# jvde-github/AIS-catcher

Hardware: NVIDIA H100
Metric: IQ MSamples/s through full 2-ch demod chain (higher is better)
Workload: dtype f32

## Files before the change

ais-catcher_b200/csrc/fe_stream.cuh:

```cuda
#pragma once
#include "exact.cuh"
#include "params.h"
#include <atomic>
#include <algorithm>

namespace aisgpu {

struct Cic5 { c64 h0, h1, h2, h3, h4; };
__device__ __forceinline__ void cic5_zero(Cic5 &s) { s.h0 = s.h1 = s.h2 = s.h3 = s.h4 = 0ull; }
__device__ __forceinline__ c64 ds2_pair(Cic5 &s, c64 xe, c64 xo, c64 sc) {
	c64 z = xe;
	const c64 r0 = z; z = padd(z, s.h0);
	const c64 r1 = z; z = padd(z, s.h1);
	const c64 r2 = z; z = padd(z, s.h2);
	const c64 r3 = z; z = padd(z, s.h3);
	const c64 r4 = z; z = padd(z, s.h4);
	const c64 out = pmul(z, sc);
	z = xo;
	s.h0 = z; z = padd(z, r0);
	s.h1 = z; z = padd(z, r1);
	s.h2 = z; z = padd(z, r2);
	s.h3 = z; z = padd(z, r3);
	s.h4 = z;
	(void)r4;
	return out;
}
__device__ __forceinline__ void fcic_pair(Cic5 &s, c64 xe, c64 xo, c64 sc, c64 &oe, c64 &oo) {
	c64 z = xe;
	const c64 r0 = z; z = padd(z, s.h0);
	const c64 r1 = z; z = padd(z, s.h1);
	const c64 r2 = z; z = padd(z, s.h2);
	const c64 r3 = z; z = padd(z, s.h3);
	const c64 r4 = z; z = padd(z, s.h4);
	oe = pmul(z, sc);
	z = xo;
	s.h0 = z; z = padd(z, r0);
	s.h1 = z; z = padd(z, r1);
	s.h2 = z; z = padd(z, r2);
	s.h3 = z; z = padd(z, r3);
	s.h4 = z; z = padd(z, r4);
	oo = pmul(z, sc);
}
struct Cic5u { uint32_t h0, h1, h2, h3, h4; };
__device__ __forceinline__ void cic5u_zero(Cic5u &s) { s.h0 = s.h1 = s.h2 = s.h3 = s.h4 = 0u; }
template <int SHIFT>
__device__ __forceinline__ uint32_t ds2u_pair(Cic5u &s, uint32_t xe, uint32_t xo) {
	constexpr uint32_t m16 = 0xFFFFu >> SHIFT, mask = m16 | (m16 << 16);
	uint32_t z = xe;
	const uint32_t r0 = z; z += s.h0;
	const uint32_t r1 = z; z += s.h1;
	const uint32_t r2 = z; z += s.h2;
	const uint32_t r3 = z; z += s.h3;
	z += s.h4;
	const uint32_t out = (z >> SHIFT) & mask;
	z = xo;
	s.h0 = z; z += r0;
	s.h1 = z; z += r1;
	s.h2 = z; z += r2;
	s.h3 = z; z += r3;
	s.h4 = z;
	return out;
}
__device__ __forceinline__ c64 u16pair_to_c64(uint32_t z) {
	z ^= 0x80008000u;
	return pack2(__fmul_rn((float)(short)(z & 0xFFFFu), 3.0517578125e-05f), __fmul_rn((float)(short)(z >> 16), 3.0517578125e-05f));
}

template <int FMT, int G>
struct StFmt {
	static constexpr int BPS = FMT == 0 ? 8 : (FMT == 3 ? 4 : 2);
	static constexpr int CHUNK = G * BPS;
	static constexpr int PIECES = CHUNK / 16;
	static constexpr int SLOT = CHUNK + 16;
};
template <int FMT>
__device__ __forceinline__ void st_read_pair(const unsigned char *slot, int j, c64 &xe, c64 &xo) {
	if (FMT == 0) {
		const ulonglong2 v = *reinterpret_cast<const ulonglong2 *>(slot + j * 16);
		xe = v.x;
		xo = v.y;
	}
	else if (FMT == 1) {
		const uchar4 v = *reinterpret_cast<const uchar4 *>(slot + j * 4);
		xe = pack2(__fmul_rn((float)((int)v.x - 128), 0.0078125f), __fmul_rn((float)((int)v.y - 128), 0.0078125f));
		xo = pack2(__fmul_rn((float)((int)v.z - 128), 0.0078125f), __fmul_rn((float)((int)v.w - 128), 0.0078125f));
	}
	else if (FMT == 2) {
		const char4 v = *reinterpret_cast<const char4 *>(slot + j * 4);
		xe = pack2(__fmul_rn((float)v.x, 0.0078125f), __fmul_rn((float)v.y, 0.0078125f));
		xo = pack2(__fmul_rn((float)v.z, 0.0078125f), __fmul_rn((float)v.w, 0.0078125f));
	}
	else {
		const short4 v = *reinterpret_cast<const short4 *>(slot + j * 8);
		xe = pack2(__fmul_rn((float)v.x, 3.0517578125e-05f), __fmul_rn((float)v.y, 3.0517578125e-05f));
		xo = pack2(__fmul_rn((float)v.z, 3.0517578125e-05f), __fmul_rn((float)v.w, 3.0517578125e-05f));
	}
}

template <int FMT, int K, int ST_G, int ST_NB, int ST_WARPS, bool PRE = false>
__global__ void __launch_bounds__(ST_WARPS * 32) k_frontend_st(const FeParams p) {
	static_assert(K >= 3 && K <= 7, "streaming front end: 768 kS/s .. 12288 kS/s");
	static_assert(ST_G <= (1 << (K + 2)) && (ST_G % 16) == 0, "a chunk must not be longer than a super-step");
	typedef StFmt<FMT, ST_G> F;
	constexpr int SS = 1 << (K + 2);
	constexpr int NCH = SS / ST_G;
	constexpr int N96 = SS >> K;
	extern __shared__ __align__(16) unsigned char st_ring[];
	const int lane = threadIdx.x & 31, wib = threadIdx.x >> 5;
	const long long g0 = ((long long)blockIdx.x * ST_WARPS + wib) * 32;
	const int L = p.st_L;
	if (g0 >= (long long)p.st_B * L) return;
	int stream = (int)((g0 + lane) / L), sub = (int)((g0 + lane) - (long long)stream * L);
	const bool ghost = stream >= p.st_B;
	if (ghost) { stream = p.st_B - 1; sub = L - 1; }
	const int n_short = L - p.st_r;
	const int n_main = ghost ? 0 : p.st_q + (sub >= n_short ? 1 : 0);
	unsigned char(*ring)[32 * F::SLOT] = reinterpret_cast<unsigned char(*)[32 * F::SLOT]>(st_ring + (size_t)wib * ST_NB * 32 * F::SLOT);
	const long long a = ((long long)sub * p.st_q + max(0, sub - n_short)) * SS;
	const int n_super = p.P / SS + p.st_q + (p.st_r ? 1 : 0);
	const int warp_chunks = n_super * NCH;
	constexpr int OWN_PER_IT = 32 / F::PIECES;
	const int o0 = lane / F::PIECES, q0 = lane % F::PIECES;
	const unsigned char *in0 = reinterpret_cast<const unsigned char *>(p.in) - (long long)p.P * F::BPS;
	const unsigned my_off = (unsigned)((((long long)stream * p.in_stride + a) * F::BPS) >> 4);
	const unsigned long long my_warm = sub == 0 ? (unsigned long long)(reinterpret_cast<const unsigned char *>(p.tail) + (long long)stream * p.P * F::BPS)
												: (unsigned long long)(in0 + ((unsigned long long)my_off << 4));
	const int dst_off = o0 * F::SLOT + q0 * 16;
	unsigned own_off[F::PIECES];
#pragma unroll
	for (int it = 0; it < F::PIECES; it++) own_off[it] = __shfl_sync(0xffffffffu, my_off, it * OWN_PER_IT + o0);
	auto prefetch = [&](int c) {
		if (c < warp_chunks) {
			const long long coff = (long long)c * (ST_G * F::BPS) + q0 * 16;
			unsigned char *dst = &ring[c % ST_NB][dst_off];
			if (c * ST_G < p.P) {
#pragma unroll 1
				for (int it = 0; it < F::PIECES; it++) {
					const unsigned long long w = __shfl_sync(0xffffffffu, my_warm, it * OWN_PER_IT + o0);
					cp_async16(dst + it * OWN_PER_IT * F::SLOT, reinterpret_cast<const unsigned char *>(w) + coff);
				}
			}
			else {
				unsigned long long base = (unsigned long long)(in0 + coff);
				asm volatile("" : "+l"(base));
#pragma unroll
				for (int it = 0; it < F::PIECES; it++) cp_async16(dst + it * OWN_PER_IT * F::SLOT, reinterpret_cast<const unsigned char *>(base + ((unsigned long long)own_off[it] << 4)));
			}
		}
		cp_async_commit();
	};
	const c64 sc = pack2(0.03125f, 0.03125f);
	static_assert(FMT != 4 || (K == 4 && !PRE), "the integer front end exists for the exact 1536K bucket only (Model.cpp:222-236)");
	Cic5 lv[K], chA, chB, fA, fB;
	Cic5u lu[4];
	uint32_t pendu[4];
#pragma unroll
	for (int l = 0; l < 4; l++) { cic5u_zero(lu[l]); pendu[l] = 0u; }
#pragma unroll
	for (int l = 0; l < K; l++) cic5_zero(lv[l]);
	cic5_zero(chA); cic5_zero(chB); cic5_zero(fA); cic5_zero(fB);
	c64 fd1 = 0ull, fd2 = 0ull;
	const float2 *rot_g = PRE ? nullptr : p.rot + (p.P >> K) + ((a - p.P) >> K);
	float2 *Cg = PRE ? p.D0 + (long long)stream * p.d0_stride + p.d0_off + ((a - p.P) >> K)
					 : p.C + (long long)(stream * 2) * p.c_stride + p.c_off + ((a - p.P) >> (K + 1));
	const int warm_super = p.P / SS;
#pragma unroll
	for (int c = 0; c < ST_NB - 1; c++) prefetch(c);
	float2 rt_n1[N96], rt_n2[N96];
#pragma unroll
	for (int i = 0; i < N96; i++) {
		rt_n1[i] = PRE ? make_float2(0.f, 0.f) : __ldg(rot_g + i);
		rt_n2[i] = PRE ? make_float2(0.f, 0.f) : __ldg(rot_g + (n_super > 1 ? N96 : 0) + i);
	}
	for (int ss = 0; ss < n_super; ss++) {
		float2 rt[N96];
#pragma unroll
		for (int i = 0; i < N96; i++) {
			rt[i] = rt_n1[i];
			rt_n1[i] = rt_n2[i];
		}
		if (!PRE && ss + 2 < n_super) {
#pragma unroll
			for (int i = 0; i < N96; i++) rt_n2[i] = __ldg(rot_g + (ss + 2) * N96 + i);
		}
		c64 lvK[N96];
		c64 pend[K + 1];
		c64 upE = 0ull, dnE = 0ull, waE = 0ull, wbE = 0ull;
		c64 outA0 = 0ull, outA1 = 0ull, outB0 = 0ull, outB1 = 0ull;
#pragma unroll
		for (int cc = 0; cc < NCH; cc++) {
			const int c = ss * NCH + cc;
			prefetch(c + ST_NB - 1);
			cp_async_wait<ST_NB - 1>();
			__syncwarp();
			{
				const unsigned char *slot = &ring[c % ST_NB][lane * F::SLOT];
#pragma unroll
				for (int j = 0; j < ST_G / 2; j++) {
					const int n1 = cc * (ST_G / 2) + j;
					c64 y = 0ull;
					int idx = n1;
					bool live = true;
					if (FMT == 4) {
						const uchar4 v = *reinterpret_cast<const uchar4 *>(slot + j * 4);
						uint32_t yu = ds2u_pair<3>(lu[0], (uint32_t)v.x | ((uint32_t)v.y << 16), (uint32_t)v.z | ((uint32_t)v.w << 16));
						if ((idx & 1) == 0) { pendu[1] = yu; live = false; }
						else { yu = ds2u_pair<4>(lu[1], pendu[1], yu); idx >>= 1; }
						if (live) {
							if ((idx & 1) == 0) { pendu[2] = yu; live = false; }
							else { yu = ds2u_pair<5>(lu[2], pendu[2], yu); idx >>= 1; }
						}
						if (live) {
							if ((idx & 1) == 0) { pendu[3] = yu; live = false; }
							else {
								y = u16pair_to_c64(ds2u_pair<0>(lu[3], pendu[3], yu));
								if (p.st_first && sub == 0 && ss < warm_super) y = 0ull;
								idx >>= 1;
							}
						}
					}
					else {
						c64 xe, xo;
						st_read_pair<FMT == 4 ? 1 : FMT>(slot, j, xe, xo);
						y = ds2_pair(lv[0], xe, xo, sc);
#pragma unroll
						for (int l = 1; l < K; l++) {
							if (live) {
								if ((idx & 1) == 0) { pend[l] = y; live = false; }
								else { y = ds2_pair(lv[l], pend[l], y, sc); idx >>= 1; }
							}
						}
					}
					if (live && PRE) lvK[idx] = y;
					if (live && !PRE) {
						c64 x = y;
						if (p.use_fdc) {
							const float2 h1 = unpack2(fd1), h2 = unpack2(fd2), yv = unpack2(y);
							const float tx = __fadd_rn(h1.x, yv.x), ty = __fadd_rn(h1.y, yv.y);
							x = pack2(__fadd_rn(__fmul_rn(p.fdc_alpha, tx), __fmul_rn(h2.x, p.fdc_beta)),
									  __fadd_rn(__fmul_rn(p.fdc_alpha, ty), __fmul_rn(h2.y, p.fdc_beta)));
							fd1 = fd2;
							fd2 = y;
						}
						const float2 xv = unpack2(x);
						const float2 r = rt[idx];
						const float RR = __fmul_rn(xv.x, r.x), II = __fmul_rn(xv.y, r.y), RI = __fmul_rn(xv.x, r.y), IR = __fmul_rn(xv.y, r.x);
						const c64 up = pack2(__fsub_rn(RR, II), __fadd_rn(IR, RI));
						const c64 dn = pack2(__fadd_rn(RR, II), __fsub_rn(IR, RI));
						if ((idx & 1) == 0) { upE = up; dnE = dn; }
						else {
							const c64 wa = ds2_pair(chA, upE, up, sc), wb = ds2_pair(chB, dnE, dn, sc);
							if ((idx & 2) == 0) { waE = wa; wbE = wb; }
							else {
								fcic_pair(fA, waE, wa, sc, outA0, outA1);
								fcic_pair(fB, wbE, wb, sc, outB0, outB1);
							}
						}
					}
				}
			}
			__syncwarp();
		}
		if (PRE) {
			if (ss >= warm_super && ss - warm_super < n_main) {
				float2 *o = Cg + ss * N96;
#pragma unroll
				for (int i = 0; i < N96; i += 2) *reinterpret_cast<ulonglong2 *>(o + i) = make_ulonglong2(lvK[i], lvK[i + 1]);
			}
		}
		else if (ss >= warm_super && ss - warm_super < n_main) {
			float2 *o = Cg + ss * 2;
			*reinterpret_cast<ulonglong2 *>(o) = make_ulonglong2(outA0, outA1);
			*reinterpret_cast<ulonglong2 *>(o + p.c_stride) = make_ulonglong2(outB0, outB1);
		}
	}
	cp_async_wait<0>();
}

static inline bool st_plan(long long B, int nss, int warm, int wpc, int slots, int min_ratio, int forced_L, int &L, int &q, int &r) {
	const int q_min = warm * min_ratio > 0 ? warm * min_ratio : 1;
	if (nss < q_min) return false;
	const int L_max = nss / q_min;
	auto cost = [&](int l) {
		const long long ctas = ((B * l + 31) / 32 + wpc - 1) / wpc;
		const long long waves = (ctas + slots - 1) / slots;
		return (double)waves * ((nss + l - 1) / l + warm);
	};
	int best = 1;
	double cb = cost(1);
	for (int l = 2; l <= L_max; l++) {
		const double c = cost(l);
		if (c < cb * 0.97) { cb = c; best = l; }
	}
	if (forced_L > 0) best = forced_L < L_max ? forced_L : L_max;
	L = best;
	q = nss / L;
	r = nss - q * L;
	return true;
}
struct CtaSlots { std::atomic<int> slots{0}, sms{0}; };
template <typename Kernel>
static cudaError_t cta_slots(CtaSlots &cache, Kernel *kernel, int threads, size_t smem, int &slots, int &sms) {
	slots = cache.slots.load();
	sms = cache.sms.load();
	if (slots) return cudaSuccess;
	int dev = 0, occ = 0;
	cudaError_t e;
	if ((e = cudaGetDevice(&dev)) != cudaSuccess) return e;
	if ((e = cudaDeviceGetAttribute(&sms, cudaDevAttrMultiProcessorCount, dev)) != cudaSuccess) return e;
	if ((e = cudaOccupancyMaxActiveBlocksPerMultiprocessor(&occ, kernel, threads, smem)) != cudaSuccess) return e;
	slots = sms * (occ > 0 ? occ : 1);
	cache.sms.store(sms);
	cache.slots.store(slots);
	return cudaSuccess;
}

template <int FMT, int K, int G, int NB, int WPC, bool PRE>
static cudaError_t launch_st_one(const FeParams &p_in, int forced_L, cudaStream_t s) {
	constexpr int GG = G <= (1 << (K + 2)) ? G : (1 << (K + 2));
	constexpr int SS = 1 << (K + 2);
	const size_t smem = (size_t)WPC * NB * 32 * StFmt<FMT, GG>::SLOT;
	cudaError_t e = cudaFuncSetAttribute(k_frontend_st<FMT, K, GG, NB, WPC, PRE>, cudaFuncAttributeMaxDynamicSharedMemorySize, (int)smem);
	if (e != cudaSuccess) return e;
	static CtaSlots cache;
	int slots = 0, sms = 0;
	if ((e = cta_slots(cache, k_frontend_st<FMT, K, GG, NB, WPC, PRE>, WPC * 32, smem, slots, sms)) != cudaSuccess) return e;
	if (p_in.st_cap > 0) slots = std::min(slots, sms * p_in.st_cap);
	FeParams p = p_in;
	if (p.N % SS || p.P % SS) return cudaErrorNotSupported;
	if ((unsigned long long)p.st_B * (unsigned long long)p.in_stride * StFmt<FMT, GG>::BPS >= (1ull << 36)) return cudaErrorNotSupported;
	if (!st_plan(p.st_B, p.N / SS, p.P / SS, WPC, slots, FMT == 4 ? 1 : 4, forced_L, p.st_L, p.st_q, p.st_r)) return cudaErrorNotSupported;
	const long long n_warps = ((long long)p.st_B * p.st_L + 31) / 32;
	const unsigned ctas = (unsigned)((n_warps + WPC - 1) / WPC);
	k_frontend_st<FMT, K, GG, NB, WPC, PRE><<<ctas, WPC * 32, smem, s>>>(p);
	return cudaGetLastError();
}
template <int FMT, int G, int NB, int WPC>
cudaError_t launch_frontend_stream_shape(const FeParams &p, int k, bool pre, int forced_L, cudaStream_t s) {
	if (pre) {
		switch (k) {
		case 3: return launch_st_one<FMT, 3, G, NB, WPC, true>(p, forced_L, s);
		case 4: return launch_st_one<FMT, 4, G, NB, WPC, true>(p, forced_L, s);
		case 5: return launch_st_one<FMT, 5, G, NB, WPC, true>(p, forced_L, s);
		default: return cudaErrorNotSupported;
		}
	}
	switch (k) {
	case 3: return launch_st_one<FMT, 3, G, NB, WPC, false>(p, forced_L, s);
	case 4: return launch_st_one<FMT, 4, G, NB, WPC, false>(p, forced_L, s);
	case 5: return launch_st_one<FMT, 5, G, NB, WPC, false>(p, forced_L, s);
	case 6: return launch_st_one<FMT, 6, G, NB, WPC, false>(p, forced_L, s);
	case 7: return launch_st_one<FMT, 7, G, NB, WPC, false>(p, forced_L, s);
	default: return cudaErrorNotSupported;
	}
}
extern template cudaError_t launch_frontend_stream_shape<0, 32, 3, 4>(const FeParams &, int, bool, int, cudaStream_t);
extern template cudaError_t launch_frontend_stream_shape<1, 16, 8, 1>(const FeParams &, int, bool, int, cudaStream_t);
extern template cudaError_t launch_frontend_stream_shape<2, 16, 8, 1>(const FeParams &, int, bool, int, cudaStream_t);
extern template cudaError_t launch_frontend_stream_shape<3, 16, 8, 1>(const FeParams &, int, bool, int, cudaStream_t);

}
```

Before: 244,700.

## Split CF32 streaming front end across thread pairs, one per I/Q component

Adds a new streaming front-end kernel for CF32 input at K=5..7 in which each stream is handled by two lanes, one for the real and one for the imaginary component. The CIC chains run on scalar floats instead of packed complex pairs, and the complex rotation is done with a lane-pair shuffle. This doubles the thread-level parallelism and warp count per CTA and shortens each thread's serial dependency chain. The cost is extra shuffles, duplicated control flow per lane, and a changed occupancy and CTA plan.

```diff
diff --git a/ais-catcher_b200/csrc/fe_stream.cuh b/ais-catcher_b200/csrc/fe_stream.cuh
--- a/ais-catcher_b200/csrc/fe_stream.cuh
+++ b/ais-catcher_b200/csrc/fe_stream.cuh
@@ -40,6 +40,40 @@
 	s.h3 = z; z = padd(z, r3);
 	s.h4 = z; z = padd(z, r4);
 	oo = pmul(z, sc);
+}
+struct Cic5s { float h0, h1, h2, h3, h4; };
+__device__ __forceinline__ void cic5s_zero(Cic5s &s) { s.h0 = s.h1 = s.h2 = s.h3 = s.h4 = 0.f; }
+__device__ __forceinline__ float ds2_one(Cic5s &s, float xe, float xo) {
+	float z = xe;
+	const float r0 = z; z = __fadd_rn(z, s.h0);
+	const float r1 = z; z = __fadd_rn(z, s.h1);
+	const float r2 = z; z = __fadd_rn(z, s.h2);
+	const float r3 = z; z = __fadd_rn(z, s.h3);
+	z = __fadd_rn(z, s.h4);
+	const float out = __fmul_rn(z, 0.03125f);
+	z = xo;
+	s.h0 = z; z = __fadd_rn(z, r0);
+	s.h1 = z; z = __fadd_rn(z, r1);
+	s.h2 = z; z = __fadd_rn(z, r2);
+	s.h3 = z; z = __fadd_rn(z, r3);
+	s.h4 = z;
+	return out;
+}
+__device__ __forceinline__ void fcic_one(Cic5s &s, float xe, float xo, float &oe, float &oo) {
+	float z = xe;
+	const float r0 = z; z = __fadd_rn(z, s.h0);
+	const float r1 = z; z = __fadd_rn(z, s.h1);
+	const float r2 = z; z = __fadd_rn(z, s.h2);
+	const float r3 = z; z = __fadd_rn(z, s.h3);
+	const float r4 = z; z = __fadd_rn(z, s.h4);
+	oe = __fmul_rn(z, 0.03125f);
+	z = xo;
+	s.h0 = z; z = __fadd_rn(z, r0);
+	s.h1 = z; z = __fadd_rn(z, r1);
+	s.h2 = z; z = __fadd_rn(z, r2);
+	s.h3 = z; z = __fadd_rn(z, r3);
+	s.h4 = z; z = __fadd_rn(z, r4);
+	oo = __fmul_rn(z, 0.03125f);
 }
 struct Cic5u { uint32_t h0, h1, h2, h3, h4; };
 __device__ __forceinline__ void cic5u_zero(Cic5u &s) { s.h0 = s.h1 = s.h2 = s.h3 = s.h4 = 0u; }
@@ -277,6 +311,145 @@
 	cp_async_wait<0>();
 }
 
+template <int K, int ST_G, int ST_NB, int ST_WARPS>
+__global__ void __launch_bounds__(ST_WARPS * 32) k_frontend_stc(const FeParams p) {
+	static_assert(K >= 3 && K <= 7, "streaming front end: 768 kS/s .. 12288 kS/s");
+	static_assert(ST_G <= (1 << (K + 2)) && (ST_G % 16) == 0, "a chunk must not be longer than a super-step");
+	typedef StFmt<0, ST_G> F;
+	constexpr int OWN = 16;
+	constexpr int SS = 1 << (K + 2);
+	constexpr int NCH = SS / ST_G;
+	constexpr int N96 = SS >> K;
+	extern __shared__ __align__(16) unsigned char st_ring[];
+	const int lane = threadIdx.x & 31, wib = threadIdx.x >> 5, own = lane >> 1, comp = lane & 1;
+	const long long g0 = ((long long)blockIdx.x * ST_WARPS + wib) * OWN;
+	const int L = p.st_L;
+	if (g0 >= (long long)p.st_B * L) return;
+	int stream = (int)((g0 + own) / L), sub = (int)((g0 + own) - (long long)stream * L);
+	const bool ghost = stream >= p.st_B;
+	if (ghost) { stream = p.st_B - 1; sub = L - 1; }
+	const int n_short = L - p.st_r;
+	const int n_main = ghost ? 0 : p.st_q + (sub >= n_short ? 1 : 0);
+	unsigned char(*ring)[OWN * F::SLOT] = reinterpret_cast<unsigned char(*)[OWN * F::SLOT]>(st_ring + (size_t)wib * ST_NB * OWN * F::SLOT);
+	const long long a = ((long long)sub * p.st_q + max(0, sub - n_short)) * SS;
+	const int n_super = p.P / SS + p.st_q + (p.st_r ? 1 : 0);
+	const int warp_chunks = n_super * NCH;
+	constexpr int OWN_PER_IT = 32 / F::PIECES;
+	constexpr int ITS = OWN / OWN_PER_IT;
+	const int o0 = lane / F::PIECES, q0 = lane % F::PIECES;
+	const unsigned char *in0 = reinterpret_cast<const unsigned char *>(p.in) - (long long)p.P * F::BPS;
+	const unsigned my_off = (unsigned)((((long long)stream * p.in_stride + a) * F::BPS) >> 4);
+	const unsigned long long my_warm = sub == 0 ? (unsigned long long)(reinterpret_cast<const unsigned char *>(p.tail) + (long long)stream * p.P * F::BPS)
+												: (unsigned long long)(in0 + ((unsigned long long)my_off << 4));
+	const int dst_off = o0 * F::SLOT + q0 * 16;
+	unsigned own_off[ITS];
+#pragma unroll
+	for (int it = 0; it < ITS; it++) own_off[it] = __shfl_sync(0xffffffffu, my_off, 2 * (it * OWN_PER_IT + o0));
+	auto prefetch = [&](int c) {
+		if (c < warp_chunks) {
+			const long long coff = (long long)c * (ST_G * F::BPS) + q0 * 16;
+			unsigned char *dst = &ring[c % ST_NB][dst_off];
+			if (c * ST_G < p.P) {
+#pragma unroll 1
+				for (int it = 0; it < ITS; it++) {
+					const unsigned long long w = __shfl_sync(0xffffffffu, my_warm, 2 * (it * OWN_PER_IT + o0));
+					cp_async16(dst + it * OWN_PER_IT * F::SLOT, reinterpret_cast<const unsigned char *>(w) + coff);
+				}
+			}
+			else {
+				unsigned long long base = (unsigned long long)(in0 + coff);
+				asm volatile("" : "+l"(base));
+#pragma unroll
+				for (int it = 0; it < ITS; it++) cp_async16(dst + it * OWN_PER_IT * F::SLOT, reinterpret_cast<const unsigned char *>(base + ((unsigned long long)own_off[it] << 4)));
+			}
+		}
+		cp_async_commit();
+	};
+	Cic5s lv[K], chA, chB, fA, fB;
+#pragma unroll
+	for (int l = 0; l < K; l++) cic5s_zero(lv[l]);
+	cic5s_zero(chA); cic5s_zero(chB); cic5s_zero(fA); cic5s_zero(fB);
+	float fd1 = 0.f, fd2 = 0.f;
+	const float2 *rot_g = p.rot + (p.P >> K) + ((a - p.P) >> K);
+	float2 *Cg = p.C + (long long)(stream * 2) * p.c_stride + p.c_off + ((a - p.P) >> (K + 1));
+	const int warm_super = p.P / SS;
+	const unsigned ysign = comp ? 0x80000000u : 0u;
+#pragma unroll
+	for (int c = 0; c < ST_NB - 1; c++) prefetch(c);
+	float2 rt_n1[N96], rt_n2[N96];
+#pragma unroll
+	for (int i = 0; i < N96; i++) {
+		rt_n1[i] = __ldg(rot_g + i);
+		rt_n2[i] = __ldg(rot_g + (n_super > 1 ? N96 : 0) + i);
+	}
+	for (int ss = 0; ss < n_super; ss++) {
+		float2 rt[N96];
+#pragma unroll
+		for (int i = 0; i < N96; i++) {
+			rt[i] = rt_n1[i];
+			rt_n1[i] = rt_n2[i];
+		}
+		if (ss + 2 < n_super) {
+#pragma unroll
+			for (int i = 0; i < N96; i++) rt_n2[i] = __ldg(rot_g + (ss + 2) * N96 + i);
+		}
+		float pend[K + 1];
+		float upE = 0.f, dnE = 0.f, waE = 0.f, wbE = 0.f;
+		float outA0 = 0.f, outA1 = 0.f, outB0 = 0.f, outB1 = 0.f;
+#pragma unroll
+		for (int cc = 0; cc < NCH; cc++) {
+			const int c = ss * NCH + cc;
+			prefetch(c + ST_NB - 1);
+			cp_async_wait<ST_NB - 1>();
+			__syncwarp();
+			{
+				const float *slot = reinterpret_cast<const float *>(&ring[c % ST_NB][own * F::SLOT]) + comp;
+#pragma unroll
+				for (int j = 0; j < ST_G / 2; j++) {
+					const int n1 = cc * (ST_G / 2) + j;
+					int idx = n1;
+					bool live = true;
+					float y = ds2_one(lv[0], slot[4 * j], slot[4 * j + 2]);
+#pragma unroll
+					for (int l = 1; l < K; l++) {
+						if (live) {
+							if ((idx & 1) == 0) { pend[l] = y; live = false; }
+							else { y = ds2_one(lv[l], pend[l], y); idx >>= 1; }
+						}
+					}
+					if (live) {
+						float x = y;
+						if (p.use_fdc) {
+							x = __fadd_rn(__fmul_rn(p.fdc_alpha, __fadd_rn(fd1, y)), __fmul_rn(fd2, p.fdc_beta));
+							fd1 = fd2;
+							fd2 = y;
+						}
+						const float xb = __shfl_xor_sync(0xffffffffu, x, 1);
+						const float2 r = rt[idx];
+						const float pa = __fmul_rn(x, r.x), pb = __fmul_rn(xb, __uint_as_float(__float_as_uint(r.y) ^ ysign));
+						const float up = __fsub_rn(pa, pb), dn = __fadd_rn(pa, pb);
+						if ((idx & 1) == 0) { upE = up; dnE = dn; }
+						else {
+							const float wa = ds2_one(chA, upE, up), wb = ds2_one(chB, dnE, dn);
+							if ((idx & 2) == 0) { waE = wa; wbE = wb; }
+							else {
+								fcic_one(fA, waE, wa, outA0, outA1);
+								fcic_one(fB, wbE, wb, outB0, outB1);
+							}
+						}
+					}
+				}
+			}
+			__syncwarp();
+		}
+		const float m0 = comp ? outB0 : outA0, m1 = comp ? outB1 : outA1;
+		const float t0 = __shfl_xor_sync(0xffffffffu, comp ? outA0 : outB0, 1), t1 = __shfl_xor_sync(0xffffffffu, comp ? outA1 : outB1, 1);
+		if (ss >= warm_super && ss - warm_super < n_main)
+			*reinterpret_cast<float4 *>(Cg + ss * 2 + (comp ? p.c_stride : 0)) = comp ? make_float4(t0, m0, t1, m1) : make_float4(m0, t0, m1, t1);
+	}
+	cp_async_wait<0>();
+}
+
 static inline bool st_plan(long long B, int nss, int warm, int wpc, int slots, int min_ratio, int forced_L, int &L, int &q, int &r) {
 	const int q_min = warm * min_ratio > 0 ? warm * min_ratio : 1;
 	if (nss < q_min) return false;
@@ -315,28 +488,35 @@
 	return cudaSuccess;
 }
 
-template <int FMT, int K, int G, int NB, int WPC, bool PRE>
+template <int FMT, int K, int G, int NB, int WPC, bool PRE, bool PAIR = false>
 static cudaError_t launch_st_one(const FeParams &p_in, int forced_L, cudaStream_t s) {
+	static_assert(!PAIR || (FMT == 0 && !PRE), "the thread-pair front end is CF32's, behind Rotate");
 	constexpr int GG = G <= (1 << (K + 2)) ? G : (1 << (K + 2));
 	constexpr int SS = 1 << (K + 2);
-	const size_t smem = (size_t)WPC * NB * 32 * StFmt<FMT, GG>::SLOT;
-	cudaError_t e = cudaFuncSetAttribute(k_frontend_st<FMT, K, GG, NB, WPC, PRE>, cudaFuncAttributeMaxDynamicSharedMemorySize, (int)smem);
+	constexpr int OWN = PAIR ? 16 : 32;
+	void (*kernel)(const FeParams);
+	if constexpr (PAIR) kernel = k_frontend_stc<K, GG, NB, WPC>;
+	else kernel = k_frontend_st<FMT, K, GG, NB, WPC, PRE>;
+	const size_t smem = (size_t)WPC * NB * OWN * StFmt<FMT, GG>::SLOT;
+	cudaError_t e = cudaFuncSetAttribute(kernel, cudaFuncAttributeMaxDynamicSharedMemorySize, (int)smem);
 	if (e != cudaSuccess) return e;
 	static CtaSlots cache;
 	int slots = 0, sms = 0;
-	if ((e = cta_slots(cache, k_frontend_st<FMT, K, GG, NB, WPC, PRE>, WPC * 32, smem, slots, sms)) != cudaSuccess) return e;
+	if ((e = cta_slots(cache, kernel, WPC * 32, smem, slots, sms)) != cudaSuccess) return e;
 	if (p_in.st_cap > 0) slots = std::min(slots, sms * p_in.st_cap);
 	FeParams p = p_in;
 	if (p.N % SS || p.P % SS) return cudaErrorNotSupported;
 	if ((unsigned long long)p.st_B * (unsigned long long)p.in_stride * StFmt<FMT, GG>::BPS >= (1ull << 36)) return cudaErrorNotSupported;
-	if (!st_plan(p.st_B, p.N / SS, p.P / SS, WPC, slots, FMT == 4 ? 1 : 4, forced_L, p.st_L, p.st_q, p.st_r)) return cudaErrorNotSupported;
-	const long long n_warps = ((long long)p.st_B * p.st_L + 31) / 32;
+	if (!st_plan(p.st_B, p.N / SS, p.P / SS, WPC * OWN / 32, slots, FMT == 4 ? 1 : 4, forced_L, p.st_L, p.st_q, p.st_r)) return cudaErrorNotSupported;
+	const long long n_warps = ((long long)p.st_B * p.st_L + OWN - 1) / OWN;
 	const unsigned ctas = (unsigned)((n_warps + WPC - 1) / WPC);
-	k_frontend_st<FMT, K, GG, NB, WPC, PRE><<<ctas, WPC * 32, smem, s>>>(p);
+	kernel<<<ctas, WPC * 32, smem, s>>>(p);
 	return cudaGetLastError();
 }
 template <int FMT, int G, int NB, int WPC>
 cudaError_t launch_frontend_stream_shape(const FeParams &p, int k, bool pre, int forced_L, cudaStream_t s) {
+	constexpr bool PAIR = FMT == 0;
+	constexpr int PW = PAIR ? 2 * WPC : WPC;
 	if (pre) {
 		switch (k) {
 		case 3: return launch_st_one<FMT, 3, G, NB, WPC, true>(p, forced_L, s);
@@ -348,9 +528,9 @@
 	switch (k) {
 	case 3: return launch_st_one<FMT, 3, G, NB, WPC, false>(p, forced_L, s);
 	case 4: return launch_st_one<FMT, 4, G, NB, WPC, false>(p, forced_L, s);
-	case 5: return launch_st_one<FMT, 5, G, NB, WPC, false>(p, forced_L, s);
-	case 6: return launch_st_one<FMT, 6, G, NB, WPC, false>(p, forced_L, s);
-	case 7: return launch_st_one<FMT, 7, G, NB, WPC, false>(p, forced_L, s);
+	case 5: return launch_st_one<FMT, 5, G, NB, PW, false, PAIR>(p, forced_L, s);
+	case 6: return launch_st_one<FMT, 6, G, NB, PW, false, PAIR>(p, forced_L, s);
+	case 7: return launch_st_one<FMT, 7, G, NB, PW, false, PAIR>(p, forced_L, s);
 	default: return cudaErrorNotSupported;
 	}
 }
```

New measurement: 243,600 (median of 6 runs). Within noise of the previous version (-0.5%).
